# vshmyhlo/retinanet-tensorflow

Measured on AMD Instinct MI355X. Metric: train images/sec (MobileNetV2-FPN RetinaNet 512x512, bs=2/GPU), higher is better.
Workload: dtype f32

## Files before the change

### include/rn_hip.h

```cpp
#ifndef RN_HIP_H
#define RN_HIP_H

#include <stddef.h>
#include <stdint.h>

#ifdef __cplusplus
extern "C" {
#endif

typedef void* rn_stream_t;

enum rn_status {
  RN_OK = 0,
  RN_EINVAL = -1,
  RN_EUNSUPPORTED = -2,
  RN_EHIP = -3,
  RN_EWORKSPACE = -4
};

enum rn_act { RN_ACT_NONE = 0, RN_ACT_RELU = 1, RN_ACT_ELU = 2, RN_ACT_RELU6 = 3, RN_ACT_SIGMOID = 4 };
enum rn_loss_mode { RN_LOSS_BCE_DICE = 0, RN_LOSS_FOCAL = 1 };
enum rn_opt { RN_OPT_MOMENTUM = 0, RN_OPT_RMSPROP = 1, RN_OPT_ADAM = 2 };

#define RN_MAX_SEG 16
// ... 356 lines not shown
  const float* g;
  int32_t g_plain;
  rn_mb_rows grows;
} rn_mb_dy;
typedef struct rn_mb_gout {
  float* out;
  const float* add1; const float* add2;
  const rn_mb_norm* norm;
  int32_t store_plain;
  rn_mb_rows grows;
  float* planes;
} rn_mb_gout;
size_t rn_mb_pointwise_bwd_rows(int n, int hw, int cin, int cout, int groups, rn_mb_rows* layout);
size_t rn_mb_pointwise_bwd_workspace(int n, int hw, int cin, int cout);
int rn_mb_pointwise_bwd(const float* x, const rn_mb_norm* in, const rn_mb_dy* dy, const float* w, float* dw, const rn_mb_gout* gout,
                        int n, int hw, int cin, int cout, void* workspace, size_t workspace_bytes, rn_stream_t stream,
                        rn_reduce_list* defer);
size_t rn_mb_depthwise_bwd_rows(int n, int h, int w, int c, int stride, int groups, rn_mb_rows* layout);
size_t rn_mb_depthwise_bwd_workspace(int n, int h, int w, int c, int stride);
int rn_mb_depthwise_bwd(const rn_mb_norm* in, const rn_mb_dy* dy, const float* w, float* dw, const rn_mb_gout* gout, int n, int h,
                        int wd, int stride, void* workspace, size_t workspace_bytes, rn_stream_t stream, rn_reduce_list* defer);
int rn_set_mb_dw_taps(int on);
int rn_get_mb_dw_taps(void);

int rn_iou(const float* a, int64_t na, const float* b, int64_t nb, int pairwise, float* out, int32_t* malformed,
           rn_stream_t stream);

int rn_anchor_assign(const float* boxes, const int32_t* class_ids, const int32_t* num_obj, int nimg, int max_obj,
                     const float* anchor_sizes, int num_anchors, int grid_h, int grid_w, int num_classes,
                     float* cls_out, float* reg_out, uint8_t* trainable_out, int32_t* argmax_out,
                     rn_stream_t stream);
#define RN_MAX_LEVELS 8
typedef struct rn_assign_level {
  const float* anchor_sizes;
  int grid_h, grid_w;
  float* cls_out;
  float* reg_out;
  uint8_t* trainable_out;
  int32_t* argmax_out;
} rn_assign_level;
int rn_anchor_assign_levels(const float* boxes, const int32_t* class_ids, const int32_t* num_obj, int nimg, int max_obj,
                            const rn_assign_level* levels, int nlevel, int num_anchors, int num_classes,
                            rn_stream_t stream);
int rn_anchor_assign_levels_pair(const float* boxes, const int32_t* class_ids, const int32_t* num_obj, int nimg, int max_obj,
                                 const rn_assign_level* levels, int nlevel, int num_anchors, int num_classes,
                                 rn_stream_t stream);
// ... 100 lines not shown
```

### retinanet-tensorflow_amd/_rn.py

```python
import ctypes as C
import os

import torch

_HERE = os.path.dirname(os.path.abspath(__file__))
LIB_PATH = os.environ.get("RN_LIB_PATH") or os.path.join(_HERE, "librn_hip.so")

MAX_SEG = 16
ACT = {None: 0, "none": 0, "linear": 0, "relu": 1, "elu": 2, "relu6": 3, "sigmoid": 4}
LOSS_MODE = {"bce_dice": 0, "focal": 1}
OPT = {"momentum": 0, "rmsprop": 1, "adam": 2}
OPT_BLOCK = 1024
LR_MAX_BOUNDARIES = 8
LOSS_STATS_HEADER = 8
API_VERSION = 415


class RnError(RuntimeError):
    pass


class LrSchedule(C.Structure):
    _fields_ = [("kind", C.c_int32), ("n_boundaries", C.c_int32), ("base_lr", C.c_double), ("warmup_factor", C.c_double),
                ("final_factor", C.c_double), ("decay_factor", C.c_double), ("warmup_steps", C.c_int64), ("total_steps", C.c_int64),
# ... 136 lines not shown
    "rn_zero", "rn_conv2d_fwd", "rn_conv2d_stats_rows", "rn_conv2d_fwd_stats", "rn_conv2d_dropout_rows", "rn_conv2d_fwd_dropout", "rn_depthwise_stats_rows", "rn_depthwise_fwd_stats", "rn_group_norm_rows_ok",
    "rn_conv2d_dgrad", "rn_conv2d_wgrad_workspace", "rn_conv2d_wgrad", "rn_conv2d_bwd",
    "rn_conv2d_bias_grad_workspace", "rn_conv2d_bias_grad", "rn_conv3x3_winograd_workspace", "rn_conv3x3_winograd",
    "rn_conv3x3_winograd_wgrad_workspace", "rn_conv3x3_winograd_wgrad", "rn_conv3x3_winograd_keep_bytes",
    "rn_conv3x3_winograd_bwd_workspace", "rn_conv3x3_winograd_bwd", "rn_flush_reductions", "rn_gemm_batched",
    "rn_winograd_bwd_products_workspace", "rn_winograd_bwd_products", "rn_wino_gn_rows", "rn_conv3x3_winograd_gn", "rn_conv3x3_winograd_gn_bwd", "rn_conv3x3_winograd_gn_bwd_wgrad", "rn_reduce_rows", "rn_resize_bilinear_normalize", "rn_resize_pair_u8",
    "rn_resize_pair_u8_augment_workspace", "rn_resize_pair_u8_augment",
    "rn_resize_pair_u8_batch", "rn_resize_pair_u8_augment_batch_workspace", "rn_resize_pair_u8_augment_batch",
    "rn_dwgn_supported", "rn_dwgn_fwd", "rn_dwgn_bwd", "rn_depthwise_fwd", "rn_depthwise_dgrad", "rn_depthwise_wgrad_workspace", "rn_depthwise_wgrad", "rn_depthwise_bwd",
    "rn_group_norm_sync_bytes", "rn_group_norm_workspace", "rn_group_norm_fwd", "rn_group_norm_bwd",
    "rn_act_fwd", "rn_act_bwd", "rn_upsample_add_fwd", "rn_upsample_add_bwd_top",
    "rn_pack_weights_f16", "rn_pack_weights_f16_bytes", "rn_cast_f32_to_f16", "rn_pad_cast_rgb_f16", "rn_conv2d_fwd_f16", "rn_conv2d_f16_fold_rows", "rn_conv2d_fwd_f16_fold", "rn_group_norm_finalize", "rn_group_norm_apply_f16", "rn_group_norm_apply_res_f16", "rn_maxpool_fwd_f16", "rn_maxpool_gn_fwd_f16", "rn_upsample_add_fwd_f16",
    "rn_act_fwd_f16", "rn_flip_width", "rn_dropout", "rn_dropout_strided", "rn_maxpool_fwd", "rn_maxpool_bwd", "rn_maxpool_bwd_arg", "rn_avgpool_fwd", "rn_avgpool_bwd",
    "rn_loss_workspace", "rn_loss_fwd", "rn_loss_bwd",
    "rn_iou", "rn_anchor_assign", "rn_anchor_assign_levels", "rn_anchor_assign_levels_pair", "rn_decode_boxes", "rn_detect_workspace", "rn_detect",
    "rn_boxes_decode", "rn_nms_classwise_workspace", "rn_nms_classwise",
    "rn_optimizer_workspace", "rn_grad_norm_l2reg", "rn_optimizer_step", "rn_counter_add", "rn_add_segs",
    "rn_mb_rows_max", "rn_mb_compact_rows_layout", "rn_mb_compact_rows", "rn_mb_pointwise_rows", "rn_mb_pointwise_fwd", "rn_mb_depthwise_rows", "rn_mb_depthwise_fwd", "rn_mb_apply",
    "rn_mb_resident_sync_bytes", "rn_mb_resident_rows", "rn_mb_resident_fwd", "rn_set_product_mode", "rn_get_product_mode",
    "rn_set_x3_bfrag", "rn_get_x3_bfrag", "rn_x3_bfrag_ok", "rn_x3_bfrag_bytes", "rn_x3_pack_bfrag", "rn_gemm_batched_bfrag", "rn_conv3x3_winograd_gn_u_bytes", "rn_conv3x3_winograd_gn_weights",
    "rn_conv2d_f16_stats_tiles", "rn_group_norm_fwd_f16_tiles",
    "rn_mb_pointwise_bwd_rows", "rn_mb_pointwise_bwd_workspace", "rn_mb_pointwise_bwd",
    "rn_mb_depthwise_bwd_rows", "rn_mb_depthwise_bwd_workspace", "rn_mb_depthwise_bwd", "rn_set_mb_dw_taps", "rn_get_mb_dw_taps",
    "rn_debug_collective_standin", "rn_optimizer_norm_pairs", "rn_optimizer_step_norm", "rn_norm_reg_finalize",
    "rn_lr_schedule_eval", "rn_optimizer_step_norm_lrdev", "rn_ema_decay_eval", "rn_optimizer_step_ema",
    "rn_accum_phase_eval", "rn_lr_schedule_eval_gated", "rn_ema_decay_eval_gated", "rn_optimizer_step_accum",
    "rn_optimizer_step_clip", "rn_grad_norm_partial",
    "rn_finite_gate_eval", "rn_optimizer_step_gated",
]


def lib():
    global _lib
    if _lib is None:
        if not os.path.exists(LIB_PATH):
            raise RnError("librn_hip.so not found at %s: build it with "
                          "`make -C retinanet-tensorflow_amd/csrc` (there is no fallback path)" % LIB_PATH)
        L = C.CDLL(LIB_PATH)
        if not hasattr(L, "rn_version") or L.rn_version() != API_VERSION:
            raise RnError("%s reports ABI version %s, these bindings need %d: rebuild it (make -C retinanet-tensorflow_amd/csrc)"
                          % (LIB_PATH, L.rn_version() if hasattr(L, "rn_version") else "none", API_VERSION))
        L.rn_last_error.restype = C.c_char_p
        L.rn_group_norm_sync_bytes.argtypes = []
        for name in ("rn_conv2d_wgrad_workspace", "rn_depthwise_wgrad_workspace", "rn_group_norm_workspace", "rn_group_norm_sync_bytes",
                     "rn_loss_workspace", "rn_detect_workspace", "rn_optimizer_workspace",
                     "rn_conv2d_bias_grad_workspace", "rn_nms_classwise_workspace", "rn_conv3x3_winograd_workspace", "rn_conv2d_fwd_workspace",
# ... 71 lines not shown
        L.rn_conv3x3_winograd_wgrad_workspace.argtypes = [C.c_void_p, C.c_int, C.c_int, C.c_int, C.c_int]
        L.rn_conv3x3_winograd_wgrad.argtypes = [C.c_void_p, C.c_int, C.c_int, C.c_int, C.c_void_p, C.c_int, C.c_int,
                                                C.c_void_p, C.c_size_t, C.c_void_p, C.c_void_p]
        L.rn_conv3x3_winograd_bwd_workspace.argtypes = [C.c_void_p] + [C.c_int] * 6
        L.rn_conv3x3_winograd_bwd.argtypes = [C.c_void_p, C.c_int, C.c_int, C.c_int, C.c_void_p, C.c_void_p, C.c_int, C.c_int,
                                              C.c_void_p, C.c_size_t, C.c_void_p, C.c_void_p, C.c_void_p]
        L.rn_conv3x3_winograd_keep_bytes.argtypes = [C.c_void_p, C.c_int, C.c_int, C.c_int, C.c_int, C.c_void_p, C.c_void_p]
        L.rn_conv3x3_winograd.argtypes = [C.c_void_p, C.c_int, C.c_int, C.c_int, C.c_void_p, C.c_void_p, C.c_int, C.c_int,
                                          C.c_void_p, C.c_size_t, C.c_void_p, C.c_void_p, C.c_void_p]
        L.rn_wino_gn_rows.argtypes = [C.c_void_p, C.c_int, C.c_int]
        L.rn_winograd_bwd_products_workspace.argtypes = [C.c_int] * 4
        L.rn_winograd_bwd_products.argtypes = [C.c_void_p] * 3 + [C.c_int] * 3 + [C.c_void_p] * 2 + [C.c_int] * 3 + \
                                              [C.c_void_p, C.c_size_t, C.c_void_p, C.c_void_p]
        L.rn_x3_bfrag_ok.argtypes = [C.c_int] * 3
        L.rn_conv2d_f16_stats_tiles.argtypes = [C.c_void_p, C.c_int, C.c_void_p, C.c_void_p]
        L.rn_group_norm_fwd_f16_tiles.argtypes = [C.c_void_p, C.c_int, C.c_void_p, C.c_void_p, C.c_void_p, C.c_void_p, C.c_void_p, C.c_void_p]
        L.rn_conv3x3_winograd_gn_u_bytes.argtypes = [C.c_int] * 3
        L.rn_conv3x3_winograd_gn_weights.argtypes = [C.c_void_p, C.c_int, C.c_int, C.c_int, C.c_void_p, C.c_size_t, C.c_void_p, C.c_void_p]
        L.rn_x3_bfrag_bytes.argtypes = [C.c_int] * 3
        L.rn_x3_pack_bfrag.argtypes = [C.c_void_p, C.c_void_p] + [C.c_int] * 4 + [C.c_void_p]
        L.rn_gemm_batched_bfrag.argtypes = [C.c_void_p] * 3 + [C.c_int] * 5 + [C.c_void_p]
        L.rn_set_x3_bfrag.argtypes = [C.c_int]
        L.rn_set_mb_dw_taps.argtypes = [C.c_int]
        L.rn_conv3x3_winograd_gn.argtypes = [C.c_void_p, C.c_int, C.c_int, C.c_int, C.c_void_p, C.c_void_p, C.c_int, C.c_void_p,
                                             C.c_void_p, C.c_size_t, C.c_void_p, C.c_void_p, C.c_void_p]
        L.rn_conv3x3_winograd_gn_bwd_wgrad.argtypes = [C.c_void_p, C.c_int, C.c_int, C.c_int, C.c_void_p, C.c_int, C.c_int, C.c_void_p, C.c_size_t,
                                                       C.c_void_p, C.c_int, C.c_void_p]
        L.rn_conv3x3_winograd_gn_bwd.argtypes = [C.c_void_p, C.c_int, C.c_int, C.c_int, C.c_void_p, C.c_void_p, C.c_int, C.c_int,
                                                 C.c_void_p, C.c_void_p, C.c_size_t, C.c_void_p, C.c_void_p, C.c_void_p]
        L.rn_reduce_rows.argtypes = [C.c_void_p, C.c_void_p, C.c_int64, C.c_int, C.c_int, C.c_void_p, C.c_void_p]
        L.rn_conv2d_bias_grad.argtypes = [C.c_void_p, C.c_int, C.c_void_p, C.c_void_p, C.c_void_p, C.c_size_t,
                                          C.c_void_p, C.c_void_p]
        L.rn_group_norm_workspace.argtypes = [C.c_void_p, C.c_int, C.c_void_p]
        L.rn_group_norm_fwd.argtypes = [C.c_void_p, C.c_int, C.c_void_p, C.c_void_p, C.c_void_p, C.c_void_p,
                                        C.c_size_t, C.c_void_p]
        L.rn_group_norm_bwd.argtypes = [C.c_void_p, C.c_int, C.c_void_p, C.c_void_p, C.c_void_p, C.c_void_p,
                                        C.c_void_p, C.c_void_p, C.c_size_t, C.c_void_p, C.c_void_p]
        L.rn_act_fwd.argtypes = [C.c_void_p, C.c_void_p, C.c_int64, C.c_int, C.c_void_p]
        L.rn_act_bwd.argtypes = [C.c_void_p, C.c_void_p, C.c_void_p, C.c_int64, C.c_int, C.c_void_p]
        L.rn_upsample_add_fwd.argtypes = [C.c_void_p] * 3 + [C.c_int] * 6 + [C.c_void_p]
        L.rn_upsample_add_bwd_top.argtypes = [C.c_void_p] * 2 + [C.c_int] * 6 + [C.c_void_p]
        L.rn_pack_weights_f16.argtypes = [C.c_void_p, C.c_void_p, C.c_int, C.c_int, C.c_int, C.c_int, C.c_void_p]
        L.rn_pack_weights_f16_bytes.argtypes = [C.c_int, C.c_int, C.c_int, C.c_int]
        L.rn_pack_weights_f16_bytes.restype = C.c_size_t
        L.rn_cast_f32_to_f16.argtypes = [C.c_void_p, C.c_void_p, C.c_int64, C.c_void_p]
        L.rn_pad_cast_rgb_f16.argtypes = [C.c_void_p, C.c_void_p, C.c_int64, C.c_void_p]
# ... 221 lines not shown
```

### retinanet-tensorflow_amd/csrc/mbconv.hip

```cpp
#include <type_traits>

#include "mb_common.h"

namespace {


template <int BM, int BN, int WM, int WN, bool NORM, int ACT, int KS, int NST>
__global__ __launch_bounds__(WM* WN * 64 * KS) void mb_pw_fwd_kernel(const PwFwdArgs a) {
  constexpr int TG = WM * WN * 64;
  constexpr bool RES = NORM && ACT != RN_ACT_ELU && ACT != RN_ACT_RELU6 && ACT != RN_ACT_RELU;
  static_assert(TG * KS >= T || !NORM, "the prologue needs 256 threads");
  constexpr int TM = BM / WM / 32, TN = BN / WN / 32;
  constexpr int KQ = BK / 4, A_RPP = TG / KQ, A_PASS = BM / A_RPP;
  constexpr int NQ = BN / 4, B_RPP = TG / NQ, B_PASS = BK / B_RPP;
  static_assert(A_PASS >= 1 && B_PASS >= 1 && BM % A_RPP == 0 && BK % B_RPP == 0, "tile/threads mismatch");
  constexpr int OPF = BM * LDK + BK * BN;
  static_assert(KS * OPF * 4 >= (T + GMAX) * 16 && OPF >= (WM + 1) * BN * 2, "operand tiles double as scratch");
  static_assert(KS == 1 || KS * OPF >= (KS - 1) * TM * TN * 16 * TG, "operand tiles double as the split-K exchange");
  __shared__ __attribute__((aligned(16))) float smem[KS * OPF];
  __shared__ __attribute__((aligned(16))) float tab[NORM ? 2 * KMAX : 4];
  __shared__ float gstat[NORM ? GMAX : 1][2];
  const int tid = threadIdx.x, grp = tid / TG, lt = tid % TG, lane = lt & 63, wave = lt >> 6;
  float* As = smem + grp * OPF;
  float* Bs = As + BM * LDK;
// ... 986 lines not shown
  }
  __syncthreads();
  if (tid < ond.groups) {
    float t1 = 0.f, t2 = 0.f;
    for (int c = tid * ond.cpg; c < (tid + 1) * ond.cpg; ++c) {
      const float w = ond.gamma[c];
      t1 += w * chan[c * 2 + 0]; t2 += w * chan[c * 2 + 1];
    }
    go.grows.rows[(size_t)prow * go.grows.W + tid] = make_float2(t1, t2);
  }
}

struct DwBwdArgs {
  int dbg;
  NormDev in; DyDev dy; const float* w; float* partial; GoutDev go;
  int n, h, wd, c, stride, oh, ow, pad_t, pad_l;
  int th, tw, tiles_h, tiles_w, sw, nslab;
  int oph, opw;
  int tpb, nblk;
};

__device__ __forceinline__ int floor_div(int a, int b) { return a >= 0 ? a / b : -((-a + b - 1) / b); }

template <int ACT, bool MULTI, int S, bool TAPS, int NPA = NP, int NPD = NP, bool PF = false>
__global__ __launch_bounds__(T, 2) void mb_dw_bwd_kernel(const DwBwdArgs a) {
  extern __shared__ __attribute__((aligned(16))) float dsm[];
  __shared__ __attribute__((aligned(16))) float tabA[4 * 128];
  __shared__ __attribute__((aligned(16))) float tabD[3 * 128];
  __shared__ __attribute__((aligned(16))) float wtab[9 * 128];
  __shared__ float gstat[GMAX][2];
  __shared__ float gc[GMAX][2];
  const int tid = threadIdx.x;
  const int bid = rn::xcd_remap(blockIdx.x, gridDim.x);
  const int slab = bid % a.nslab;
  const int tt = bid / a.nslab;
  const int ntile = a.tiles_h * a.tiles_w;
  const int blk = tt % a.nblk, sample = tt / a.nblk;
  const int tile_lo = MULTI ? blk * a.tpb : blk, tile_hi = MULTI ? min(tile_lo + a.tpb, ntile) : tile_lo + 1;
  const int C = a.c, SW = a.sw, SQ = SW >> 2, c0 = slab * SW;
  constexpr int s = S;
  const int tw_shift = 31 - __builtin_clz(a.tw);
  const int aph = a.th + 2, apw = a.tw + 2;
  float* a1p = dsm;
  float* dyp = dsm + (size_t)aph * apw * SW;
  const int g0 = c0 / a.in.cpg, ng = SW / a.in.cpg;
  ChanPre<1> pre_a, pre_d;
  prefetch_chan<1>(a.in.gamma, a.in.beta, c0, SW, tid, pre_a);
  prefetch_chan<1>(a.dy.nd.gamma, nullptr, c0, SW, tid, pre_d);
  const GroupPre gp_a = prefetch_groups(a.in, sample, g0, ng, tid);
  const GroupPre gp_d = prefetch_groups(a.dy.nd, sample, g0, ng, tid);
  const int atotal = aph * apw * SQ;
  const int dtotal = a.oph * a.opw * SQ;
  const __amdgpu_buffer_rsrc_t xs = make_rsrc(a.in.y + (size_t)sample * a.h * a.wd * C + c0, (unsigned)(a.h * a.wd * C - c0) * 4u);
  const __amdgpu_buffer_rsrc_t gs = make_rsrc(a.dy.g + (size_t)sample * a.oh * a.ow * C + c0, (unsigned)(a.oh * a.ow * C - c0) * 4u);
  const __amdgpu_buffer_rsrc_t ys = make_rsrc(a.dy.nd.y + (size_t)sample * a.oh * a.ow * C + c0, (unsigned)(a.oh * a.ow * C - c0) * 4u);
  float4 av[NPA], gv[NPD], yv2[NPD];
  int pka[NPA], pkd[NPD];
#pragma unroll
  for (int j = 0; j < NPA; ++j) pka[j] = patch_pack(tid + j * T, atotal, SQ, apw);
#pragma unroll
  for (int j = 0; j < NPD; ++j) pkd[j] = patch_pack(tid + j * T, dtotal, SQ, a.opw);
  auto load_patches = [&](int tile) {
    const int ih0 = (tile / a.tiles_w) * a.th, iw0 = (tile % a.tiles_w) * a.tw;
    const int ay0 = ih0 - a.pad_t, ax0 = iw0 - a.pad_l;
#pragma unroll
    for (int j = 0; j < NPA; ++j) {
      const PatchElem e = patch_at(pka[j], ay0, ax0, a.h, a.wd);
// ... 6 lines not shown
      const unsigned off = (e.live && e.inside) ? ((unsigned)e.pix * C + e.q * 4) * 4u : OOB;
      gv[j] = Vec<4>::load(gs, off);
      yv2[j] = Vec<4>::load(ys, off);
    }
  };
  load_patches(tile_lo);
  const int lanes = T / SQ, q4 = tid % SQ, pl = tid / SQ;
  const bool active = pl < lanes;
  float4 wv[9];
  if (MULTI) {
    for (int e = tid; e < 9 * SQ; e += T)
      *reinterpret_cast<float4*>(&wtab[(e / SQ) * 128 + (e % SQ) * 4]) = *reinterpret_cast<const float4*>(a.w + (size_t)(e / SQ) * C + c0 + (e % SQ) * 4);
  } else {
#pragma unroll
    for (int t = 0; t < 9; ++t) wv[t] = *reinterpret_cast<const float4*>(a.w + (size_t)t * C + c0 + q4 * 4);
  }
  dy_table(a.dy, sample, a.oh * a.ow, c0, SW, dsm, gstat, gc, tabD, 128, gp_d, pre_d, tid);
  group_stats(a.in, sample, a.h * a.wd, g0, ng, false, dsm, gstat, gp_a, tid);
  scale_shift_table(a.in, c0, SW, g0, gstat, tabA, tabA + 128, pre_a, tid);
  for (int i = tid; i < SW; i += T) {
    const int g = (c0 + i) / a.in.cpg - g0;
    tabA[256 + i] = gstat[g][0]; tabA[384 + i] = gstat[g][1];
  }
  __syncthreads();
  if (a.dbg == 1) { if (av[0].x == 123.456f && gv[0].x == 1.f && yv2[0].x == 1.f) a.go.out[0] = 0.f; return; }
  const bool drop = a.in.drop_rate > 0.f;
  const uint64_t seed = a.in.seed + (a.in.seed_dev ? *a.in.seed_dev : 0ull);
  const uint64_t samp_off = (uint64_t)sample * a.h * a.wd * C;
  float s1[4] = {0.f, 0.f, 0.f, 0.f}, s2[4] = {0.f, 0.f, 0.f, 0.f};
  float4 wacc[9];
#pragma unroll
  for (int t = 0; t < 9; ++t) wacc[t] = make_float4(0.f, 0.f, 0.f, 0.f);
  const float* __restrict__ y1 = a.in.y + (size_t)sample * a.h * a.wd * C + c0 + q4 * 4;
  float* __restrict__ go = a.go.out + (size_t)sample * a.h * a.wd * C + c0 + q4 * 4;
  auto process_tile = [&](int tile) {
    const int ih0 = (tile / a.tiles_w) * a.th, iw0 = (tile % a.tiles_w) * a.tw;
    const int ay0 = ih0 - a.pad_t, ax0 = iw0 - a.pad_l;
    const int oy0 = floor_div(ih0 + a.pad_t - 2 + (s - 1), s), ox0 = floor_div(iw0 + a.pad_l - 2 + (s - 1), s);
#pragma unroll
    for (int j = 0; j < NPA; ++j) {
      const PatchElem e = patch_at(pka[j], ay0, ax0, a.h, a.wd);
      if (e.live) {
        float4 o = norm_act_drop<ACT>(av[j], *reinterpret_cast<const float4*>(&tabA[e.q * 4]), *reinterpret_cast<const float4*>(&tabA[128 + e.q * 4]),
                                      a.in.act, drop, a.in.drop_rate, a.in.keep_scale, seed, samp_off + (uint64_t)e.pix * C + c0 + e.q * 4);
        if (!e.inside) o = make_float4(0.f, 0.f, 0.f, 0.f);
        *reinterpret_cast<float4*>(&a1p[(size_t)(tid + j * T) * 4]) = o;
      }
    }
#pragma unroll
    for (int j = 0; j < NPD; ++j) {
      const PatchElem e = patch_at(pkd[j], oy0, ox0, a.oh, a.ow);
      if (e.live) {
        float4 o = dy_of(gv[j], yv2[j], tabD, 128, e.q * 4, false, 0.f, 1.f, 0ull, 0ull);
        if (!e.inside) o = make_float4(0.f, 0.f, 0.f, 0.f);
        *reinterpret_cast<float4*>(&dyp[(size_t)(tid + j * T) * 4]) = o;
      }
    }
    __syncthreads();
    if (PF && tile + 1 < tile_hi) load_patches(tile + 1);
    if (active) {
      const float4 sc = *reinterpret_cast<const float4*>(&tabA[q4 * 4]), sh = *reinterpret_cast<const float4*>(&tabA[128 + q4 * 4]);
      const float4 mn = *reinterpret_cast<const float4*>(&tabA[256 + q4 * 4]), rs = *reinterpret_cast<const float4*>(&tabA[384 + q4 * 4]);
      auto g1_of = [&](int ih, int iw, const float4 yv, const float4 acc) {
        const float yy[4] = {yv.x, yv.y, yv.z, yv.w}, dd[4] = {acc.x, acc.y, acc.z, acc.w};
        const float scv[4] = {sc.x, sc.y, sc.z, sc.w}, shv[4] = {sh.x, sh.y, sh.z, sh.w};
        const float mnv[4] = {mn.x, mn.y, mn.z, mn.w}, rsv[4] = {rs.x, rs.y, rs.z, rs.w};
        float g[4], mk[4] = {1.f, 1.f, 1.f, 1.f};
        if (drop) keep4(seed, samp_off + (uint64_t)(ih * a.wd + iw) * C + c0 + q4 * 4, a.in.drop_rate, a.in.keep_scale, mk);
#pragma unroll
        for (int j = 0; j < 4; ++j) {
          const float z = fmaf(yy[j], scv[j], shv[j]);
          const float xh = (yy[j] - mnv[j]) * rsv[j];
          const float t = dd[j] * actgrad_of<ACT>(z, a.in.act) * mk[j];
          g[j] = t;
          s1[j] += t; s2[j] = fmaf(t, xh, s2[j]);
        }
        *reinterpret_cast<float4*>(go + (size_t)(ih * a.wd + iw) * C) = make_float4(g[0], g[1], g[2], g[3]);
      };
      auto tap_w = [&](int t) { return MULTI ? *reinterpret_cast<const float4*>(&wtab[t * 128 + q4 * 4]) : wv[t]; };
      const float* __restrict__ dq = dyp + q4 * 4;
      const int drow = a.opw * SW;
      if constexpr (!TAPS) {
        for (int p = pl; p < a.th * a.tw; p += lanes) {
          const int ty = p >> tw_shift, tx = p - (ty << tw_shift);
          const int ih = ih0 + ty, iw = iw0 + tx;
          if (ih < a.h && iw < a.wd) {
            const float4 yv = *reinterpret_cast<const float4*>(y1 + (size_t)(ih * a.wd + iw) * C);
            float4 acc = make_float4(0.f, 0.f, 0.f, 0.f);
#pragma unroll
            for (int kh = 0; kh < 3; ++kh) {
              const int ohs = ih + a.pad_t - kh;
              const int oh_ = S == 1 ? ohs : (ohs >> 1);
              const bool rok = ohs >= 0 && oh_ * s == ohs && oh_ < a.oh;
              const int py = min(max(oh_ - oy0, 0), a.oph - 1);
#pragma unroll
              for (int kw = 0; kw < 3; ++kw) {
                const int ows = iw + a.pad_l - kw;
                const int ow_ = S == 1 ? ows : (ows >> 1);
                const float m = (rok && ows >= 0 && ow_ * s == ows && ow_ < a.ow) ? 1.f : 0.f;
                const int px = min(max(ow_ - ox0, 0), a.opw - 1);
                const float4 dv = *reinterpret_cast<const float4*>(&dyp[((size_t)py * a.opw + px) * SW + q4 * 4]);
                const float4 w4 = tap_w(kh * 3 + kw);
                acc.x = fmaf(dv.x * m, w4.x, acc.x); acc.y = fmaf(dv.y * m, w4.y, acc.y);
                acc.z = fmaf(dv.z * m, w4.z, acc.z); acc.w = fmaf(dv.w * m, w4.w, acc.w);
              }
            }
            g1_of(ih, iw, yv, acc);
          }
        }
      } else if constexpr (S == 1) {
        for (int p = pl; p < a.th * a.tw; p += lanes) {
          const int ty = p >> tw_shift, tx = p - (ty << tw_shift);
          const int ih = ih0 + ty, iw = iw0 + tx;
          if (ih < a.h && iw < a.wd) {
            const float4 yv = *reinterpret_cast<const float4*>(y1 + (size_t)(ih * a.wd + iw) * C);
            const float* b = dq + (ty * a.opw + tx) * SW;
            float4 acc = make_float4(0.f, 0.f, 0.f, 0.f);
#pragma unroll
            for (int kh = 0; kh < 3; ++kh)
#pragma unroll
              for (int kw = 0; kw < 3; ++kw) {
                const float4 dv = *reinterpret_cast<const float4*>(b + (2 - kh) * drow + (2 - kw) * SW);
                const float4 w4 = tap_w(kh * 3 + kw);
                acc.x = fmaf(dv.x, w4.x, acc.x); acc.y = fmaf(dv.y, w4.y, acc.y);
                acc.z = fmaf(dv.z, w4.z, acc.z); acc.w = fmaf(dv.w, w4.w, acc.w);
              }
            g1_of(ih, iw, yv, acc);
          }
        }
      } else {
        auto taps_of = [&](auto cy_, auto cx_, const float* b, float4& acc) {
          constexpr int CY = decltype(cy_)::value, CX = decltype(cx_)::value;
#pragma unroll
          for (int kh = CY; kh < 3; kh += 2)
#pragma unroll
            for (int kw = CX; kw < 3; kw += 2) {
              const float4 dv = *reinterpret_cast<const float4*>(b + ((2 - kh) >> 1) * drow + ((2 - kw) >> 1) * SW);
              const float4 w4 = tap_w(kh * 3 + kw);
              acc.x = fmaf(dv.x, w4.x, acc.x); acc.y = fmaf(dv.y, w4.y, acc.y);
              acc.z = fmaf(dv.z, w4.z, acc.z); acc.w = fmaf(dv.w, w4.w, acc.w);
            }
        };
        using I0 = std::integral_constant<int, 0>;
        using I1 = std::integral_constant<int, 1>;
        for (int p = pl; p < a.th * a.tw; p += lanes) {
          const int ty = p >> tw_shift, tx = p - (ty << tw_shift);
          const int ih = ih0 + ty, iw = iw0 + tx;
          if (ih < a.h && iw < a.wd) {
            const float4 yv = *reinterpret_cast<const float4*>(y1 + (size_t)(ih * a.wd + iw) * C);
            const int cy = (ty + a.pad_t) & 1, cx = (tx + a.pad_l) & 1;
            const int py = ((ty + a.pad_t - cy) >> 1) - a.pad_t + cy, px = ((tx + a.pad_l - cx) >> 1) - a.pad_l + cx;
            const float* b = dq + (py * a.opw + px) * SW;
            float4 acc = make_float4(0.f, 0.f, 0.f, 0.f);
            if (cy == 0) {
              if (cx == 0) taps_of(I0{}, I0{}, b, acc); else taps_of(I0{}, I1{}, b, acc);
            } else {
              if (cx == 0) taps_of(I1{}, I0{}, b, acc); else taps_of(I1{}, I1{}, b, acc);
            }
            g1_of(ih, iw, yv, acc);
          }
        }
      }
    }
    if (active) {
      const int oyb = ih0 / s, oxb = iw0 / s;
      if constexpr (!TAPS) {
        const int noy = (a.th + s - 1) / s, nox = (a.tw + s - 1) / s;
        for (int p = pl; p < noy * nox; p += lanes) {
          const int ty = p / nox, tx = p - ty * nox;
          const int oh_ = oyb + ty, ow_ = oxb + tx;
          if (oh_ < a.oh && ow_ < a.ow) {
            const float4 dv = *reinterpret_cast<const float4*>(&dyp[((size_t)(oh_ - oy0) * a.opw + (ow_ - ox0)) * SW + q4 * 4]);
#pragma unroll
            for (int kh = 0; kh < 3; ++kh)
#pragma unroll
              for (int kw = 0; kw < 3; ++kw) {
                const float4 xv = *reinterpret_cast<const float4*>(&a1p[((size_t)(ty * s + kh) * apw + tx * s + kw) * SW + q4 * 4]);
                float4& t = wacc[kh * 3 + kw];
                t.x = fmaf(xv.x, dv.x, t.x); t.y = fmaf(xv.y, dv.y, t.y); t.z = fmaf(xv.z, dv.z, t.z); t.w = fmaf(xv.w, dv.w, t.w);
              }
          }
        }
// ... 39 lines not shown
  }
#pragma unroll
  for (int j = 0; j < 4; ++j) { red[tid * RW + 36 + j] = s1[j]; red[tid * RW + 40 + j] = s2[j]; }
  __syncthreads();
  float* chan = dsm + T * RW;
  const int brow = sample * a.nblk + blk;
  for (int e = tid; e < 11 * SW; e += T) {
    const int k = e / SW, ch = e - k * SW;
    const int qd = ch >> 2, comp = ch & 3;
    float t = 0.f;
    for (int l = 0; l < lanes; ++l) t += red[(l * SQ + qd) * RW + k * 4 + comp];
    if (k < 9) {
      a.partial[((size_t)brow * 9 + k) * C + c0 + ch] = t;
    } else {
      chan[ch * 2 + (k - 9)] = t;
      a.go.planes[(size_t)(k - 9) * a.go.plane_stride + (size_t)brow * C + c0 + ch] = t;
    }
  }
  __syncthreads();
  const int cpg = a.in.cpg;
  if (tid < ng) {
    float t1 = 0.f, t2 = 0.f;
    for (int j = 0; j < cpg; ++j) {
      const float w = a.in.gamma[c0 + tid * cpg + j];
      t1 += w * chan[(tid * cpg + j) * 2 + 0]; t2 += w * chan[(tid * cpg + j) * 2 + 1];
    }
    a.go.grows.rows[(size_t)brow * a.go.grows.W + g0 + tid] = make_float2(t1, t2);
  }
}

int g_dw_taps = -1;
int dw_taps_on() {
  if (g_dw_taps < 0) g_dw_taps = !(getenv("RN_MB_DW_TAPS") && atoi(getenv("RN_MB_DW_TAPS")) == 0);
  return g_dw_taps;
}

}

extern "C" int rn_set_mb_dw_taps(int on) {
  g_dw_taps = on ? 1 : 0;
  return RN_OK;
}
extern "C" int rn_get_mb_dw_taps(void) { return dw_taps_on(); }

extern "C" size_t rn_mb_pointwise_rows(int n, int hw, int cin, int cout, int groups, rn_mb_rows* layout) {
  if (n < 1 || hw < 1 || cin < 4 || cout < 4 || groups < 1 || cout % groups) return 0;
  const PwCfg c = pw_cfg(n, hw, cin, cout);
  if (hw % c.bm) return 0;
  const int R = hw / c.bm, W = groups + rn::ceil_div(cout, c.bn);
  if (cout / groups > c.bn) return 0;
  if (layout) { layout->rows_per_sample = R; layout->width = W; layout->bn = c.bn; }
  return (size_t)n * R * W * 8;
}

extern "C" int rn_mb_pointwise_fwd(const float* x, const rn_mb_norm* in, const float* residual, float* materialise, const float* w, float* y,
                                   int n, int hw, int cin, int cout, const rn_mb_rows* stat_out, int stat_groups, rn_stream_t stream) {
  RN_CHECK_ARG((x != nullptr) != (in != nullptr), "mb pointwise fwd: exactly one of x / in");
  RN_CHECK_ARG(w && y && n >= 1 && hw >= 1, "mb pointwise fwd: bad argument");
  RN_UNSUPPORTED(cin % 4 || cout % 4 || cin > KMAX || cout > KMAX, "mb pointwise fwd: cin=%d cout=%d (multiples of 4, <= %d)", cin, cout, KMAX);
  RN_UNSUPPORTED((double)n * hw * cin >= 536870912.0 || (double)n * hw * cout >= 536870912.0, "mb pointwise fwd: tensor >= 2 GiB");
  RN_CHECK_ARG(in || (!residual && !materialise), "mb pointwise fwd: residual / materialise come with `in`");
  PwFwdArgs a = {};
  a.dbg = dbg_word("pwf");
  a.x = x; a.res = residual; a.mat = materialise; a.w = w; a.y = y;
  a.n = n; a.hw = hw; a.cin = cin; a.cout = cout;
  if (in) {
// ... 186 lines not shown
}
struct DwBwdPlan { int th, tw, tiles_h, tiles_w, sw, nslab, oph, opw, tpb, nblk; };
bool dw_bwd_plan(int n, int h, int w, int c, int stride, int cpg, DwBwdPlan* p) {
  p->sw = dw_slab(c, cpg);
  if (!p->sw) return false;
  p->nslab = c / p->sw;
  static const int th_big = getenv("RN_MB_DWB_TH") ? atoi(getenv("RN_MB_DWB_TH")) : 8;
  static const int tw_big = getenv("RN_MB_DWB_TW") ? atoi(getenv("RN_MB_DWB_TW")) : 8;
  const bool big = (long)h * w >= 16384;
  int th = big ? th_big : 8, tw = big ? tw_big : 8;
  auto blocks = [&]() { return (long)n * rn::ceil_div(h, th) * rn::ceil_div(w, tw) * p->nslab; };
  auto too_big = [&]() { return (long)(th + 2) * (tw + 2) * (p->sw / 4) > NP * T || (long)(th / stride + 2) * (tw / stride + 2) * (p->sw / 4) > NP * T; };
  while ((blocks() < 384 && th * tw > 16) || (too_big() && th * tw > 16)) {
    if (th >= tw) th /= 2; else tw /= 2;
  }
  p->th = th; p->tw = tw;
  p->tiles_h = rn::ceil_div(h, th); p->tiles_w = rn::ceil_div(w, tw);
  p->oph = th / stride + 2; p->opw = tw / stride + 2;
  if ((long)(th + 2) * (tw + 2) * (p->sw / 4) > NP * T || (long)p->oph * p->opw * (p->sw / 4) > NP * T) return false;
  p->tpb = dw_tiles_per_block(blocks(), p->tiles_h * p->tiles_w);
  p->nblk = rn::ceil_div(p->tiles_h * p->tiles_w, p->tpb);
  return true;
}
size_t dw_bwd_lds_bytes(const DwBwdPlan& p) {
  size_t patches = ((size_t)(p.th + 2) * (p.tw + 2) + (size_t)p.oph * p.opw) * p.sw * 4;
  size_t scratch = (size_t)(T + GMAX) * 16;
  size_t red = (size_t)(T * 44 + 2 * p.sw) * 4;
  size_t m = patches > scratch ? patches : scratch;
  return m > red ? m : red;
}
}

extern "C" size_t rn_mb_pointwise_bwd_rows(int n, int hw, int cin, int cout, int groups, rn_mb_rows* layout) {
  if (n < 1 || hw < 1 || cin < 4 || cout < 4 || groups < 1 || cin % groups || hw % 64) return 0;
  PwBigCfg big;
  if (pw_big_cfg(n, hw, cin, cout, &big)) {
    if (layout) { layout->rows_per_sample = big.bps; layout->width = groups + 1; layout->bn = big.nti * 16; }
    return (size_t)n * big.bps * (groups + 1) * 8;
  }
  const int pb = pw_bwd_cfg(n, hw, cin, cout).dpb;
  const int R = hw / pb, W = groups + rn::ceil_div(cin, pb);
  if (cin / groups > pb) return 0;
  if (layout) { layout->rows_per_sample = R; layout->width = W; layout->bn = pb; }
  return (size_t)n * R * W * 8;
}
extern "C" size_t rn_mb_pointwise_bwd_workspace(int n, int hw, int cin, int cout) {
  if (n < 1 || hw < 64 || hw % 64 || cin < 4 || cout < 4) return 0;
  PwBigCfg big;
// ... 112 lines not shown
  DwBwdArgs a = {};
  a.dbg = dbg_word("dwb");
  if (int e = fill_norm(in, &a.in, n, false, "mb depthwise bwd")) return e;
  a.in.st.rows = nullptr;
  const int c = in->c;
  RN_UNSUPPORTED((double)n * h * wd * c >= 536870912.0, "mb depthwise bwd: tensor >= 2 GiB");
  if (int e = fill_dy(dy, &a.dy, n, c, "mb depthwise bwd")) return e;
  RN_CHECK_ARG(!a.dy.g_plain && dy->norm->groups == in->groups, "mb depthwise bwd: the GroupNorms around a depthwise conv share their grouping");
  a.w = w; a.n = n; a.h = h; a.wd = wd; a.c = c; a.stride = stride;
  rn::same_pad(h, 3, stride, &a.oh, &a.pad_t);
  rn::same_pad(wd, 3, stride, &a.ow, &a.pad_l);
  DwBwdPlan p;
  RN_UNSUPPORTED(!dw_bwd_plan(n, h, wd, c, stride, a.in.cpg, &p), "mb depthwise bwd: no channel slab for c=%d groups=%d", c, in->groups);
  a.th = p.th; a.tw = p.tw; a.tiles_h = p.tiles_h; a.tiles_w = p.tiles_w; a.sw = p.sw; a.nslab = p.nslab; a.oph = p.oph; a.opw = p.opw;
  a.tpb = p.tpb; a.nblk = p.nblk;
  rn_mb_rows want = {};
  RN_UNSUPPORTED(!rn_mb_depthwise_bwd_rows(n, h, wd, c, stride, in->groups, &want), "mb depthwise bwd: this shape cannot emit gradient rows");
  if (int e = fill_gout(gout, &a.go, n, c, want, "mb depthwise bwd")) return e;
  RN_CHECK_ARG(gout->norm->y == in->y, "mb depthwise bwd: gout->norm is the block of `in`");
  const int nrows = n * p.nblk;
  const size_t need = (size_t)nrows * 9 * c * sizeof(float);
  if (workspace_bytes < need) { rn::set_error("mb depthwise bwd: workspace %zu < %zu bytes", workspace_bytes, need); return RN_EWORKSPACE; }
  a.partial = (float*)workspace;
  const size_t lds = dw_bwd_lds_bytes(p);
  RN_UNSUPPORTED(lds > 64 * 1024, "mb depthwise bwd: patches of %zu bytes", lds);
  const dim3 grid((unsigned)((long)nrows * p.nslab));
  hipStream_t st = (hipStream_t)stream;
  RN_CHECK_ARG((p.tw & (p.tw - 1)) == 0 && (p.th & (p.th - 1)) == 0 && p.th >= stride && p.tw >= stride,
               "mb depthwise bwd: tile %d x %d is not a power of two", p.th, p.tw);
  const bool taps = dw_taps_on();
#define RN_DWB_S(ACT_, MULTI_, S_, ...)                                                                                \
  do {                                                                                                                 \
    if (taps) hipLaunchKernelGGL((mb_dw_bwd_kernel<ACT_, MULTI_, S_, true, ##__VA_ARGS__>), grid, dim3(T), lds, st, a); \
    else hipLaunchKernelGGL((mb_dw_bwd_kernel<ACT_, MULTI_, S_, false, ##__VA_ARGS__>), grid, dim3(T), lds, st, a);    \
  } while (0)
#define RN_DWB(ACT_, MULTI_)                                                                                           \
  do {                                                                                                                 \
    if (stride == 1) RN_DWB_S(ACT_, MULTI_, 1);                                                                        \
    else RN_DWB_S(ACT_, MULTI_, 2);                                                                                    \
  } while (0)
  static const bool pf_on = !(getenv("RN_MB_DWB_PF") && atoi(getenv("RN_MB_DWB_PF")) == 0);
  const int npa = rn::ceil_div((p.th + 2) * (p.tw + 2) * (p.sw / 4), T), npd = rn::ceil_div(p.oph * p.opw * (p.sw / 4), T);
  if (in->act == RN_ACT_ELU && p.tpb > 1 && pf_on && stride == 1 && npa <= 4 && npd <= 4) RN_DWB_S(RN_ACT_ELU, true, 1, 4, 4, true);
  else if (in->act == RN_ACT_ELU && p.tpb > 1 && pf_on && stride == 1 && npa <= 5 && npd <= 5) RN_DWB_S(RN_ACT_ELU, true, 1, 5, 5, true);
  else if (in->act == RN_ACT_ELU && p.tpb > 1 && pf_on && stride == 2 && npa <= 4 && npd <= 2) RN_DWB_S(RN_ACT_ELU, true, 2, 4, 2, true);
  else if (in->act == RN_ACT_ELU && p.tpb > 1 && pf_on && stride == 2 && npa <= 5 && npd <= 2) RN_DWB_S(RN_ACT_ELU, true, 2, 5, 2, true);
  else if (in->act == RN_ACT_ELU && p.tpb == 1) RN_DWB(RN_ACT_ELU, false);
  else if (in->act == RN_ACT_ELU) RN_DWB(RN_ACT_ELU, true);
  else if (in->act == RN_ACT_RELU6) RN_DWB(RN_ACT_RELU6, true);
  else RN_DWB(-1, true);
#undef RN_DWB
#undef RN_DWB_S
  RN_LAUNCH_CHECK();
  return rn::launch_reduce_rows((const float*)workspace, dw, (int64_t)9 * c, nrows, 0, st);
}

extern "C" int rn_mb_rows_max(void) { return RMAX; }

extern "C" size_t rn_mb_compact_rows_layout(int n, const rn_mb_rows* in, rn_mb_rows* out) {
  if (!in || !out || n < 1 || in->rows_per_sample < 1 || in->width < 1 || in->width > T) return 0;
  const int F = rn::ceil_div(in->rows_per_sample, 8);
  out->rows_per_sample = rn::ceil_div(in->rows_per_sample, F); out->width = in->width; out->bn = in->bn;
  return (size_t)n * out->rows_per_sample * out->width * 8;
}

extern "C" int rn_mb_compact_rows(const rn_mb_rows* in, const rn_mb_rows* out, int n, rn_stream_t stream) {
  RN_CHECK_ARG(in && out && in->rows && out->rows && n >= 1, "mb compact rows: bad argument");
  rn_mb_rows want = {};
  RN_CHECK_ARG(rn_mb_compact_rows_layout(n, in, &want) && want.rows_per_sample == out->rows_per_sample && want.width == out->width && want.bn == out->bn,
               "mb compact rows: `out` layout differs from rn_mb_compact_rows_layout");
  CompactArgs a = {(const float2*)in->rows, (float2*)out->rows, in->rows_per_sample, in->width, rn::ceil_div(in->rows_per_sample, 8), want.rows_per_sample};
  hipLaunchKernelGGL(mb_compact_rows_kernel, dim3((unsigned)a.Rout, (unsigned)n), dim3(T), 0, (hipStream_t)stream, a);
// ... 4 lines not shown
```

Baseline: 499.8.

## Compute activation and its gradient in one pass in depthwise backward

```diff
diff --git a/include/rn_hip.h b/include/rn_hip.h
--- a/include/rn_hip.h
+++ b/include/rn_hip.h
@@ -402,6 +402,8 @@
                         int wd, int stride, void* workspace, size_t workspace_bytes, rn_stream_t stream, rn_reduce_list* defer);
 int rn_set_mb_dw_taps(int on);
 int rn_get_mb_dw_taps(void);
+int rn_set_mb_bwd_once(int on);
+int rn_get_mb_bwd_once(void);
 
 int rn_iou(const float* a, int64_t na, const float* b, int64_t nb, int pairwise, float* out, int32_t* malformed,
            rn_stream_t stream);
diff --git a/retinanet-tensorflow_amd/_rn.py b/retinanet-tensorflow_amd/_rn.py
--- a/retinanet-tensorflow_amd/_rn.py
+++ b/retinanet-tensorflow_amd/_rn.py
@@ -182,6 +182,7 @@
     "rn_conv2d_f16_stats_tiles", "rn_group_norm_fwd_f16_tiles",
     "rn_mb_pointwise_bwd_rows", "rn_mb_pointwise_bwd_workspace", "rn_mb_pointwise_bwd",
     "rn_mb_depthwise_bwd_rows", "rn_mb_depthwise_bwd_workspace", "rn_mb_depthwise_bwd", "rn_set_mb_dw_taps", "rn_get_mb_dw_taps",
+    "rn_set_mb_bwd_once", "rn_get_mb_bwd_once",
     "rn_debug_collective_standin", "rn_optimizer_norm_pairs", "rn_optimizer_step_norm", "rn_norm_reg_finalize",
     "rn_lr_schedule_eval", "rn_optimizer_step_norm_lrdev", "rn_ema_decay_eval", "rn_optimizer_step_ema",
     "rn_accum_phase_eval", "rn_lr_schedule_eval_gated", "rn_ema_decay_eval_gated", "rn_optimizer_step_accum",
@@ -299,6 +300,7 @@
         L.rn_gemm_batched_bfrag.argtypes = [C.c_void_p] * 3 + [C.c_int] * 5 + [C.c_void_p]
         L.rn_set_x3_bfrag.argtypes = [C.c_int]
         L.rn_set_mb_dw_taps.argtypes = [C.c_int]
+        L.rn_set_mb_bwd_once.argtypes = [C.c_int]
         L.rn_conv3x3_winograd_gn.argtypes = [C.c_void_p, C.c_int, C.c_int, C.c_int, C.c_void_p, C.c_void_p, C.c_int, C.c_void_p,
                                              C.c_void_p, C.c_size_t, C.c_void_p, C.c_void_p, C.c_void_p]
         L.rn_conv3x3_winograd_gn_bwd_wgrad.argtypes = [C.c_void_p, C.c_int, C.c_int, C.c_int, C.c_void_p, C.c_int, C.c_int, C.c_void_p, C.c_size_t,
diff --git a/retinanet-tensorflow_amd/csrc/mbconv.hip b/retinanet-tensorflow_amd/csrc/mbconv.hip
--- a/retinanet-tensorflow_amd/csrc/mbconv.hip
+++ b/retinanet-tensorflow_amd/csrc/mbconv.hip
@@ -1032,12 +1032,36 @@
 
 __device__ __forceinline__ int floor_div(int a, int b) { return a >= 0 ? a / b : -((-a + b - 1) / b); }
 
-template <int ACT, bool MULTI, int S, bool TAPS, int NPA = NP, int NPD = NP, bool PF = false>
+template <int ACT>
+__device__ __forceinline__ float4 norm_act_drop_grad(float4 v, float4 sc, float4 sh, int act_rt, bool drop, float rate, float keep, uint64_t seed,
+                                                     uint64_t eidx, float4& dact) {
+  const float z[4] = {fmaf(v.x, sc.x, sh.x), fmaf(v.y, sc.y, sh.y), fmaf(v.z, sc.z, sh.z), fmaf(v.w, sc.w, sh.w)};
+  float o[4], g[4];
+#pragma unroll
+  for (int j = 0; j < 4; ++j) { o[j] = act_of<ACT>(z[j], act_rt); g[j] = actgrad_of<ACT>(z[j], act_rt); }
+  if (drop) {
+    float m[4];
+    keep4(seed, eidx, rate, keep, m);
+#pragma unroll
+    for (int j = 0; j < 4; ++j) {
+      o[j] *= m[j];
+      if (m[j] == 0.f) g[j] = __uint_as_float(__float_as_uint(g[j]) | 0x80000000u);
+    }
+  }
+  dact = make_float4(g[0], g[1], g[2], g[3]);
+  return make_float4(o[0], o[1], o[2], o[3]);
+}
+
+constexpr int DWB_TABA = 4 * 128, DWB_TABD = 3 * 128, DWB_WTAB = 9 * 128, DWB_GAM = 128;
+constexpr size_t DWB_STATIC_LDS = (size_t)(DWB_TABA + DWB_TABD + DWB_WTAB + DWB_GAM + 4 * GMAX) * 4;
+
+template <int ACT, bool MULTI, int S, bool TAPS, bool ONCE, int NPA = NP, int NPD = NP, bool PF = false>
 __global__ __launch_bounds__(T, 2) void mb_dw_bwd_kernel(const DwBwdArgs a) {
+  static_assert(TAPS || !ONCE, "the one-pass activation comes with the new tap loops only");
   extern __shared__ __attribute__((aligned(16))) float dsm[];
-  __shared__ __attribute__((aligned(16))) float tabA[4 * 128];
-  __shared__ __attribute__((aligned(16))) float tabD[3 * 128];
-  __shared__ __attribute__((aligned(16))) float wtab[9 * 128];
+  __shared__ __attribute__((aligned(16))) float tabA[DWB_TABA + (ONCE ? DWB_GAM : 0)];
+  __shared__ __attribute__((aligned(16))) float tabD[DWB_TABD];
+  __shared__ __attribute__((aligned(16))) float wtab[DWB_WTAB];
   __shared__ float gstat[GMAX][2];
   __shared__ float gc[GMAX][2];
   const int tid = threadIdx.x;
@@ -1053,6 +1077,8 @@
   const int aph = a.th + 2, apw = a.tw + 2;
   float* a1p = dsm;
   float* dyp = dsm + (size_t)aph * apw * SW;
+  float* dap = dyp + (size_t)a.oph * a.opw * SW;
+  float* xhp = dap + (size_t)a.th * a.tw * SW;
   const int g0 = c0 / a.in.cpg, ng = SW / a.in.cpg;
   ChanPre<1> pre_a, pre_d;
   prefetch_chan<1>(a.in.gamma, a.in.beta, c0, SW, tid, pre_a);
@@ -1105,6 +1131,7 @@
     const int g = (c0 + i) / a.in.cpg - g0;
     tabA[256 + i] = gstat[g][0]; tabA[384 + i] = gstat[g][1];
   }
+  if (ONCE && tid < SW) tabA[DWB_TABA + tid] = pre_a.g[0];
   __syncthreads();
   if (a.dbg == 1) { if (av[0].x == 123.456f && gv[0].x == 1.f && yv2[0].x == 1.f) a.go.out[0] = 0.f; return; }
   const bool drop = a.in.drop_rate > 0.f;
@@ -1120,25 +1147,42 @@
     const int ih0 = (tile / a.tiles_w) * a.th, iw0 = (tile % a.tiles_w) * a.tw;
     const int ay0 = ih0 - a.pad_t, ax0 = iw0 - a.pad_l;
     const int oy0 = floor_div(ih0 + a.pad_t - 2 + (s - 1), s), ox0 = floor_div(iw0 + a.pad_l - 2 + (s - 1), s);
+    auto dy_pass = [&]() {
+#pragma unroll
+      for (int j = 0; j < NPD; ++j) {
+        const PatchElem e = patch_at(pkd[j], oy0, ox0, a.oh, a.ow);
+        if (e.live) {
+          float4 o = dy_of(gv[j], yv2[j], tabD, 128, e.q * 4, false, 0.f, 1.f, 0ull, 0ull);
+          if (!e.inside) o = make_float4(0.f, 0.f, 0.f, 0.f);
+          *reinterpret_cast<float4*>(&dyp[(size_t)(tid + j * T) * 4]) = o;
+        }
+      }
+    };
 #pragma unroll
     for (int j = 0; j < NPA; ++j) {
       const PatchElem e = patch_at(pka[j], ay0, ax0, a.h, a.wd);
       if (e.live) {
-        float4 o = norm_act_drop<ACT>(av[j], *reinterpret_cast<const float4*>(&tabA[e.q * 4]), *reinterpret_cast<const float4*>(&tabA[128 + e.q * 4]),
-                                      a.in.act, drop, a.in.drop_rate, a.in.keep_scale, seed, samp_off + (uint64_t)e.pix * C + c0 + e.q * 4);
+        float4 o;
+        if constexpr (ONCE) {
+          float4 da;
+          o = norm_act_drop_grad<ACT>(av[j], *reinterpret_cast<const float4*>(&tabA[e.q * 4]), *reinterpret_cast<const float4*>(&tabA[128 + e.q * 4]),
+                                      a.in.act, drop, a.in.drop_rate, a.in.keep_scale, seed, samp_off + (uint64_t)e.pix * C + c0 + e.q * 4, da);
+          const int ty = ((pka[j] >> 8) & 255) - a.pad_t, tx = ((pka[j] >> 16) & 255) - a.pad_l;
+          if ((unsigned)ty < (unsigned)a.th && (unsigned)tx < (unsigned)a.tw) {
+            const float4 mn = *reinterpret_cast<const float4*>(&tabA[256 + e.q * 4]), rs = *reinterpret_cast<const float4*>(&tabA[384 + e.q * 4]);
+            const int slot = ((ty << tw_shift) + tx) * SW + e.q * 4;
+            *reinterpret_cast<float4*>(&dap[slot]) = da;
+            *reinterpret_cast<float4*>(&xhp[slot]) = make_float4((av[j].x - mn.x) * rs.x, (av[j].y - mn.y) * rs.y, (av[j].z - mn.z) * rs.z, (av[j].w - mn.w) * rs.w);
+          }
+        } else {
+          o = norm_act_drop<ACT>(av[j], *reinterpret_cast<const float4*>(&tabA[e.q * 4]), *reinterpret_cast<const float4*>(&tabA[128 + e.q * 4]),
+                                 a.in.act, drop, a.in.drop_rate, a.in.keep_scale, seed, samp_off + (uint64_t)e.pix * C + c0 + e.q * 4);
+        }
         if (!e.inside) o = make_float4(0.f, 0.f, 0.f, 0.f);
         *reinterpret_cast<float4*>(&a1p[(size_t)(tid + j * T) * 4]) = o;
       }
     }
-#pragma unroll
-    for (int j = 0; j < NPD; ++j) {
-      const PatchElem e = patch_at(pkd[j], oy0, ox0, a.oh, a.ow);
-      if (e.live) {
-        float4 o = dy_of(gv[j], yv2[j], tabD, 128, e.q * 4, false, 0.f, 1.f, 0ull, 0ull);
-        if (!e.inside) o = make_float4(0.f, 0.f, 0.f, 0.f);
-        *reinterpret_cast<float4*>(&dyp[(size_t)(tid + j * T) * 4]) = o;
-      }
-    }
+    dy_pass();
     __syncthreads();
     if (PF && tile + 1 < tile_hi) load_patches(tile + 1);
     if (active) {
@@ -1159,6 +1203,29 @@
           s1[j] += t; s2[j] = fmaf(t, xh, s2[j]);
         }
         *reinterpret_cast<float4*>(go + (size_t)(ih * a.wd + iw) * C) = make_float4(g[0], g[1], g[2], g[3]);
+      };
+      auto g1_once = [&](int ih, int iw, int p, const float4 acc) {
+        const float4 da = *reinterpret_cast<const float4*>(&dap[p * SW + q4 * 4]), x4 = *reinterpret_cast<const float4*>(&xhp[p * SW + q4 * 4]);
+        const float dd[4] = {acc.x, acc.y, acc.z, acc.w}, dav[4] = {da.x, da.y, da.z, da.w}, xhv[4] = {x4.x, x4.y, x4.z, x4.w};
+        float g[4];
+#pragma unroll
+        for (int j = 0; j < 4; ++j) {
+          const uint32_t bits = __float_as_uint(dav[j]);
+          const float mk = (bits >> 31) ? 0.f : a.in.keep_scale;
+          const float xh = xhv[j];
+          const float t = dd[j] * __uint_as_float(bits & 0x7fffffffu) * mk;
+          g[j] = t;
+          s1[j] += t; s2[j] = fmaf(t, xh, s2[j]);
+        }
+        *reinterpret_cast<float4*>(go + (size_t)(ih * a.wd + iw) * C) = make_float4(g[0], g[1], g[2], g[3]);
+      };
+      auto y1_of = [&](int ih, int iw) {
+        if constexpr (ONCE) return make_float4(0.f, 0.f, 0.f, 0.f);
+        else return *reinterpret_cast<const float4*>(y1 + (size_t)(ih * a.wd + iw) * C);
+      };
+      auto g1_at = [&](int ih, int iw, int p, const float4 yv, const float4 acc) {
+        if constexpr (ONCE) g1_once(ih, iw, p, acc);
+        else g1_of(ih, iw, yv, acc);
       };
       auto tap_w = [&](int t) { return MULTI ? *reinterpret_cast<const float4*>(&wtab[t * 128 + q4 * 4]) : wv[t]; };
       const float* __restrict__ dq = dyp + q4 * 4;
@@ -1196,7 +1263,7 @@
           const int ty = p >> tw_shift, tx = p - (ty << tw_shift);
           const int ih = ih0 + ty, iw = iw0 + tx;
           if (ih < a.h && iw < a.wd) {
-            const float4 yv = *reinterpret_cast<const float4*>(y1 + (size_t)(ih * a.wd + iw) * C);
+            const float4 yv = y1_of(ih, iw);
             const float* b = dq + (ty * a.opw + tx) * SW;
             float4 acc = make_float4(0.f, 0.f, 0.f, 0.f);
 #pragma unroll
@@ -1208,7 +1275,7 @@
                 acc.x = fmaf(dv.x, w4.x, acc.x); acc.y = fmaf(dv.y, w4.y, acc.y);
                 acc.z = fmaf(dv.z, w4.z, acc.z); acc.w = fmaf(dv.w, w4.w, acc.w);
               }
-            g1_of(ih, iw, yv, acc);
+            g1_at(ih, iw, p, yv, acc);
           }
         }
       } else {
@@ -1230,7 +1297,7 @@
           const int ty = p >> tw_shift, tx = p - (ty << tw_shift);
           const int ih = ih0 + ty, iw = iw0 + tx;
           if (ih < a.h && iw < a.wd) {
-            const float4 yv = *reinterpret_cast<const float4*>(y1 + (size_t)(ih * a.wd + iw) * C);
+            const float4 yv = y1_of(ih, iw);
             const int cy = (ty + a.pad_t) & 1, cx = (tx + a.pad_l) & 1;
             const int py = ((ty + a.pad_t - cy) >> 1) - a.pad_t + cy, px = ((tx + a.pad_l - cx) >> 1) - a.pad_l + cx;
             const float* b = dq + (py * a.opw + px) * SW;
@@ -1240,7 +1307,7 @@
             } else {
               if (cx == 0) taps_of(I1{}, I0{}, b, acc); else taps_of(I1{}, I1{}, b, acc);
             }
-            g1_of(ih, iw, yv, acc);
+            g1_at(ih, iw, p, yv, acc);
           }
         }
       }
@@ -1326,7 +1393,7 @@
   if (tid < ng) {
     float t1 = 0.f, t2 = 0.f;
     for (int j = 0; j < cpg; ++j) {
-      const float w = a.in.gamma[c0 + tid * cpg + j];
+      const float w = ONCE ? tabA[DWB_TABA + tid * cpg + j] : a.in.gamma[c0 + tid * cpg + j];
       t1 += w * chan[(tid * cpg + j) * 2 + 0]; t2 += w * chan[(tid * cpg + j) * 2 + 1];
     }
     a.go.grows.rows[(size_t)brow * a.go.grows.W + g0 + tid] = make_float2(t1, t2);
@@ -1338,6 +1405,11 @@
   if (g_dw_taps < 0) g_dw_taps = !(getenv("RN_MB_DW_TAPS") && atoi(getenv("RN_MB_DW_TAPS")) == 0);
   return g_dw_taps;
 }
+int g_bwd_once = -1;
+int bwd_once_on() {
+  if (g_bwd_once < 0) g_bwd_once = !(getenv("RN_MB_BWD_ONCE") && atoi(getenv("RN_MB_BWD_ONCE")) == 0);
+  return g_bwd_once;
+}
 
 }
 
@@ -1346,6 +1418,11 @@
   return RN_OK;
 }
 extern "C" int rn_get_mb_dw_taps(void) { return dw_taps_on(); }
+extern "C" int rn_set_mb_bwd_once(int on) {
+  g_bwd_once = on ? 1 : 0;
+  return RN_OK;
+}
+extern "C" int rn_get_mb_bwd_once(void) { return bwd_once_on(); }
 
 extern "C" size_t rn_mb_pointwise_rows(int n, int hw, int cin, int cout, int groups, rn_mb_rows* layout) {
   if (n < 1 || hw < 1 || cin < 4 || cout < 4 || groups < 1 || cout % groups) return 0;
@@ -1578,8 +1655,8 @@
   p->nblk = rn::ceil_div(p->tiles_h * p->tiles_w, p->tpb);
   return true;
 }
-size_t dw_bwd_lds_bytes(const DwBwdPlan& p) {
-  size_t patches = ((size_t)(p.th + 2) * (p.tw + 2) + (size_t)p.oph * p.opw) * p.sw * 4;
+size_t dw_bwd_lds_bytes(const DwBwdPlan& p, bool once) {
+  size_t patches = ((size_t)(p.th + 2) * (p.tw + 2) + (size_t)p.oph * p.opw + (once ? (size_t)2 * p.th * p.tw : 0)) * p.sw * 4;
   size_t scratch = (size_t)(T + GMAX) * 16;
   size_t red = (size_t)(T * 44 + 2 * p.sw) * 4;
   size_t m = patches > scratch ? patches : scratch;
@@ -1738,32 +1815,41 @@
   const size_t need = (size_t)nrows * 9 * c * sizeof(float);
   if (workspace_bytes < need) { rn::set_error("mb depthwise bwd: workspace %zu < %zu bytes", workspace_bytes, need); return RN_EWORKSPACE; }
   a.partial = (float*)workspace;
-  const size_t lds = dw_bwd_lds_bytes(p);
-  RN_UNSUPPORTED(lds > 64 * 1024, "mb depthwise bwd: patches of %zu bytes", lds);
+  const bool taps = dw_taps_on();
+  static const bool pf_on = !(getenv("RN_MB_DWB_PF") && atoi(getenv("RN_MB_DWB_PF")) == 0);
+  const int npa = rn::ceil_div((p.th + 2) * (p.tw + 2) * (p.sw / 4), T), npd = rn::ceil_div(p.oph * p.opw * (p.sw / 4), T);
+  const bool pf = in->act == RN_ACT_ELU && p.tpb > 1 && pf_on && npa <= 5 && npd <= (stride == 1 ? 5 : 2);
+  const bool once = taps && bwd_once_on() && (pf || p.tpb == 1) && dw_bwd_lds_bytes(p, true) + DWB_STATIC_LDS <= 80 * 1024;
+  const size_t lds = dw_bwd_lds_bytes(p, once);
+  RN_UNSUPPORTED(dw_bwd_lds_bytes(p, false) > 64 * 1024, "mb depthwise bwd: patches of %zu bytes", lds);
   const dim3 grid((unsigned)((long)nrows * p.nslab));
   hipStream_t st = (hipStream_t)stream;
   RN_CHECK_ARG((p.tw & (p.tw - 1)) == 0 && (p.th & (p.th - 1)) == 0 && p.th >= stride && p.tw >= stride,
                "mb depthwise bwd: tile %d x %d is not a power of two", p.th, p.tw);
-  const bool taps = dw_taps_on();
-#define RN_DWB_S(ACT_, MULTI_, S_, ...)                                                                                \
+#define RN_DWB_S(ACT_, MULTI_, S_, ONCE_, ...)                                                                         \
   do {                                                                                                                 \
-    if (taps) hipLaunchKernelGGL((mb_dw_bwd_kernel<ACT_, MULTI_, S_, true, ##__VA_ARGS__>), grid, dim3(T), lds, st, a); \
-    else hipLaunchKernelGGL((mb_dw_bwd_kernel<ACT_, MULTI_, S_, false, ##__VA_ARGS__>), grid, dim3(T), lds, st, a);    \
+    if (once && ONCE_) {                                                                                               \
+      static const bool attr_ = hipFuncSetAttribute((const void*)mb_dw_bwd_kernel<ACT_, MULTI_, S_, true, ONCE_, ##__VA_ARGS__>,         \
+                                                    hipFuncAttributeMaxDynamicSharedMemorySize, (int)(80 * 1024 - DWB_STATIC_LDS)) == hipSuccess; \
+      RN_UNSUPPORTED(lds > 64 * 1024 && !attr_, "mb depthwise bwd: %zu bytes of LDS per block refused", lds);          \
+      hipLaunchKernelGGL((mb_dw_bwd_kernel<ACT_, MULTI_, S_, true, ONCE_, ##__VA_ARGS__>), grid, dim3(T), lds, st, a); \
+    } else if (taps) hipLaunchKernelGGL((mb_dw_bwd_kernel<ACT_, MULTI_, S_, true, false, ##__VA_ARGS__>), grid, dim3(T), lds, st, a); \
+    else hipLaunchKernelGGL((mb_dw_bwd_kernel<ACT_, MULTI_, S_, false, false, ##__VA_ARGS__>), grid, dim3(T), lds, st, a); \
   } while (0)
 #define RN_DWB(ACT_, MULTI_)                                                                                           \
   do {                                                                                                                 \
-    if (stride == 1) RN_DWB_S(ACT_, MULTI_, 1);                                                                        \
-    else RN_DWB_S(ACT_, MULTI_, 2);                                                                                    \
+    if (stride == 1) RN_DWB_S(ACT_, MULTI_, 1, !MULTI_);                                                               \
+    else RN_DWB_S(ACT_, MULTI_, 2, !MULTI_);                                                                           \
   } while (0)
-  static const bool pf_on = !(getenv("RN_MB_DWB_PF") && atoi(getenv("RN_MB_DWB_PF")) == 0);
-  const int npa = rn::ceil_div((p.th + 2) * (p.tw + 2) * (p.sw / 4), T), npd = rn::ceil_div(p.oph * p.opw * (p.sw / 4), T);
-  if (in->act == RN_ACT_ELU && p.tpb > 1 && pf_on && stride == 1 && npa <= 4 && npd <= 4) RN_DWB_S(RN_ACT_ELU, true, 1, 4, 4, true);
-  else if (in->act == RN_ACT_ELU && p.tpb > 1 && pf_on && stride == 1 && npa <= 5 && npd <= 5) RN_DWB_S(RN_ACT_ELU, true, 1, 5, 5, true);
-  else if (in->act == RN_ACT_ELU && p.tpb > 1 && pf_on && stride == 2 && npa <= 4 && npd <= 2) RN_DWB_S(RN_ACT_ELU, true, 2, 4, 2, true);
-  else if (in->act == RN_ACT_ELU && p.tpb > 1 && pf_on && stride == 2 && npa <= 5 && npd <= 2) RN_DWB_S(RN_ACT_ELU, true, 2, 5, 2, true);
+  if (pf && stride == 1 && npa <= 4 && npd <= 4) RN_DWB_S(RN_ACT_ELU, true, 1, true, 4, 4, true);
+  else if (pf && stride == 1) RN_DWB_S(RN_ACT_ELU, true, 1, true, 5, 5, true);
+  else if (pf && stride == 2 && npa <= 4) RN_DWB_S(RN_ACT_ELU, true, 2, true, 4, 2, true);
+  else if (pf && stride == 2) RN_DWB_S(RN_ACT_ELU, true, 2, true, 5, 2, true);
   else if (in->act == RN_ACT_ELU && p.tpb == 1) RN_DWB(RN_ACT_ELU, false);
   else if (in->act == RN_ACT_ELU) RN_DWB(RN_ACT_ELU, true);
+  else if (in->act == RN_ACT_RELU6 && once) RN_DWB(RN_ACT_RELU6, false);
   else if (in->act == RN_ACT_RELU6) RN_DWB(RN_ACT_RELU6, true);
+  else if (once) RN_DWB(-1, false);
   else RN_DWB(-1, true);
 #undef RN_DWB
 #undef RN_DWB_S
```

Measured after the change: 500.0 (median of 4 runs). About the same (+0.0%).
